# Raph1821/Matcha-TTS-etu-UPMC-ENSAM

Hardware: AMD Instinct MI355X
Metric: training utterances/sec (whole node) + maximum_path Mcells/sec, LJSpeech batch=32 (higher is better)
Workload: dtype bf16; 1 GPU; MatchaTTS train step (encoder + MAS + CFM decoder fwd/bwd + clip + AdamW), B=32/GPU, Tx=120, Ty=600, 80 mels; model=MatchaTTS(n_vocab=150, out_channels=80, hidden_channels=192), global_batch=32, seq_len=600, text_len=120, parallelism=dp1, precision=bf16-parity, hip_graph=True, weight_planes=2, text_encoder_forward=fp32fwd (backward bf16)

## Files before the change

### matcha-tts-etu-upmc-ensam_amd/csrc/losses.hip

```cpp
#include <hip/hip_runtime.h>

#include <cmath>
#include <cstdint>

#include "mtts_common.h"

namespace {

constexpr int kLT = 64;
constexpr int kLThreads = 256;
constexpr int kLMaxC = 128;
constexpr int kLPitch = kLMaxC + 1;

__device__ __forceinline__ float block_sum(float v, float *red) {
#pragma unroll
    for (int off = 32; off > 0; off >>= 1) v += __shfl_xor(v, off);
    __syncthreads();
    if ((threadIdx.x & 63) == 0) red[threadIdx.x >> 6] = v;
    __syncthreads();
    float s = 0.f;
    if (threadIdx.x == 0) {
#pragma unroll
        for (int i = 0; i < kLThreads / 64; ++i) s += red[i];
    }
    return s;
}

__global__ __launch_bounds__(kLThreads) void loss_partials_kernel(const float *__restrict__ u_pred,
                                                                   const float *__restrict__ x1,
                                                                   const float *__restrict__ z,
                                                                   const float *__restrict__ y,
                                                                   const float *__restrict__ mu_y,
                                                                   const float *__restrict__ mask, int C,
                                                                   int T, float one_minus_sigma,
                                                                   float *__restrict__ partials) {
    __shared__ float su[kLT * kLPitch];
    __shared__ float red[kLThreads / 64];
    const int b = blockIdx.y, t0 = blockIdx.x * kLT;
    const int nt = min(kLT, T - t0);
    const float *mb = mask + (size_t)b * T + t0;
    const size_t cm = (size_t)b * C * T;
    float d_acc = 0.f, p_acc = 0.f;
    if (u_pred) {
        const float *ub = u_pred + ((size_t)b * T + t0) * C;
#pragma unroll 4
        for (int e = threadIdx.x; e < nt * C; e += kLThreads) {
            const int tl = e / C, c = e - tl * C;
            su[tl * kLPitch + c] = ub[e];
        }
        __syncthreads();
    }
#pragma unroll 4
    for (int e = threadIdx.x; e < C * kLT; e += kLThreads) {
        const int c = e / kLT, tl = e - c * kLT;
        if (tl >= nt) continue;
        const size_t i = cm + (size_t)c * T + t0 + tl;
        if (u_pred) {
            const float u = x1[i] - one_minus_sigma * z[i];
            const float d = su[tl * kLPitch + c] - u;
            d_acc = fmaf(d, d, d_acc);
        }
        if (mu_y) {
            const float d = y[i] - mu_y[i];
            p_acc += 0.5f * (d * d + 1.8378770664093453f) * mb[tl];
        }
    }
    const float ds = block_sum(d_acc, red);
    const float ps = block_sum(p_acc, red);
    if (threadIdx.x == 0) {
        const size_t blk = (size_t)blockIdx.y * gridDim.x + blockIdx.x;
        partials[2 * blk] = ds;
        partials[2 * blk + 1] = ps;
    }
}

__global__ __launch_bounds__(kLThreads) void loss_finalize_kernel(const float *__restrict__ partials, int nblk,
                                                                   const float *__restrict__ mask, int BT,
                                                                   int C, float *__restrict__ out) {
    __shared__ float red[kLThreads / 64];
    float d = 0.f, p = 0.f, m = 0.f;
    for (int i = threadIdx.x; i < nblk; i += kLThreads) {
        d += partials[2 * i];
        p += partials[2 * i + 1];
    }
    for (int i = threadIdx.x; i < BT; i += kLThreads) m += mask[i];
    d = block_sum(d, red);
    p = block_sum(p, red);
    m = block_sum(m, red);
    if (threadIdx.x == 0) {
        const float denom = m * (float)C;
        out[0] = d / denom;
        out[1] = p / denom;
        out[2] = denom;
    }
}

__global__ __launch_bounds__(kLThreads) void loss_bwd_kernel(const float *__restrict__ g_diff,
                                                              const float *__restrict__ g_prior,
                                                              const float *__restrict__ denom_p,
                                                              const float *__restrict__ u_pred,
                                                              const float *__restrict__ x1, const float *__restrict__ z,
                                                              const float *__restrict__ y,
                                                              const float *__restrict__ mu_y,
                                                              const float *__restrict__ mask, int C, int T,
                                                              float one_minus_sigma, float *__restrict__ du_pred,
                                                              float *__restrict__ dmu_y) {
    __shared__ float su[kLT * kLPitch];
    const int b = blockIdx.y, t0 = blockIdx.x * kLT;
    const int nt = min(kLT, T - t0);
    const float *mb = mask + (size_t)b * T + t0;
    const size_t cm = (size_t)b * C * T;
    const float denom = denom_p[0];
    if (du_pred) {
    #pragma unroll 4
    for (int e = threadIdx.x; e < C * kLT; e += kLThreads) {
            const int c = e / kLT, tl = e - c * kLT;
            if (tl < nt) {
                const size_t i = cm + (size_t)c * T + t0 + tl;
                su[tl * kLPitch + c] = x1[i] - one_minus_sigma * z[i];
            }
        }
        __syncthreads();
        const float g = 2.f * g_diff[0] / denom;
        const size_t tb = ((size_t)b * T + t0) * C;
#pragma unroll 4
        for (int e = threadIdx.x; e < nt * C; e += kLThreads) {
            const int tl = e / C, c = e - tl * C;
            du_pred[tb + e] = g * (u_pred[tb + e] - su[tl * kLPitch + c]);
        }
    }
    if (dmu_y) {
        const float g = -g_prior[0] / denom;
    #pragma unroll 4
    for (int e = threadIdx.x; e < C * kLT; e += kLThreads) {
            const int c = e / kLT, tl = e - c * kLT;
            if (tl >= nt) continue;
            const size_t i = cm + (size_t)c * T + t0 + tl;
            dmu_y[i] = g * (y[i] - mu_y[i]) * mb[tl];
        }
    }
}

}

extern "C" size_t mtts_losses_workspace_size(int32_t B, int32_t T) {
    if (B < 0 || T < 0) return 0;
    return (size_t)B * ((T + kLT - 1) / kLT) * 2 * sizeof(float);
}

extern "C" int mtts_losses_fwd(const float *u_pred, const float *x1, const float *z, const float *y,
                               const float *mu_y, const float *mask, int32_t B, int32_t C, int32_t T,
                               float sigma_min, float *out, void *workspace, size_t workspace_bytes,
                               void *hip_stream) {
    MTTS_CHECK_ARG(mask && out && B >= 1 && T >= 1 && C >= 1 && B <= 65535, "losses_fwd: bad args");
    MTTS_CHECK_ARG(C <= kLMaxC, "losses_fwd: C > 128");
    MTTS_CHECK_ARG(!u_pred || (x1 && z), "losses_fwd: the CFM loss needs x1 and z");
    MTTS_CHECK_ARG(!mu_y || y, "losses_fwd: the prior loss needs y");
    if (!workspace || workspace_bytes < mtts_losses_workspace_size(B, T))
        return mtts::fail(MTTS_ERR_WORKSPACE, "losses_fwd: workspace too small");
    hipStream_t st = static_cast<hipStream_t>(hip_stream);
    dim3 grid((T + kLT - 1) / kLT, B);
    float *part = static_cast<float *>(workspace);
    hipLaunchKernelGGL(loss_partials_kernel, grid, dim3(kLThreads), 0, st, u_pred, x1, z, y, mu_y, mask, C, T,
                       (float)(1.0 - (double)sigma_min), part);
    int rc = mtts::check_launch("loss_partials_kernel");
    if (rc) return rc;
    hipLaunchKernelGGL(loss_finalize_kernel, dim3(1), dim3(kLThreads), 0, st, part, (int)(grid.x * grid.y), mask,
                       B * T, C, out);
    return mtts::check_launch("loss_finalize_kernel");
}

extern "C" int mtts_losses_bwd(const float *g_diff, const float *g_prior, const float *fwd_out, const float *u_pred, const float *x1,
                               const float *z, const float *y, const float *mu_y, const float *mask,
                               int32_t B, int32_t C, int32_t T, float sigma_min, float *du_pred, float *dmu_y,
                               void *hip_stream) {
    MTTS_CHECK_ARG(fwd_out && mask && B >= 1 && T >= 1 && C >= 1 && B <= 65535 && C <= kLMaxC,
                   "losses_bwd: bad args");
    MTTS_CHECK_ARG(!du_pred || (g_diff && u_pred && x1 && z), "losses_bwd: du_pred needs g_diff, u_pred, x1, z");
    MTTS_CHECK_ARG(!dmu_y || (g_prior && y && mu_y), "losses_bwd: dmu_y needs g_prior, y, mu_y");
    if (!du_pred && !dmu_y) return MTTS_OK;
    dim3 grid((T + kLT - 1) / kLT, B);
    hipLaunchKernelGGL(loss_bwd_kernel, grid, dim3(kLThreads), 0, static_cast<hipStream_t>(hip_stream), g_diff,
                       g_prior, fwd_out + 2, u_pred, x1, z, y, mu_y, mask, C, T, (float)(1.0 - (double)sigma_min), du_pred,
                       dmu_y);
    return mtts::check_launch("loss_bwd_kernel");
}

namespace {

constexpr int kGThreads = 1024;

__global__ __launch_bounds__(256) void sequence_mask_kernel(const int64_t *__restrict__ lengths, int B, int T,
                                                            float *__restrict__ mask, float *__restrict__ key_bias) {
    const int64_t i = (int64_t)blockIdx.x * 256 + threadIdx.x;
    if (i >= (int64_t)B * T) return;
    const int b = (int)(i / T), t = (int)(i - (int64_t)b * T);
    const float m = (int64_t)t < lengths[b] ? 1.f : 0.f;
    if (mask) mask[i] = m;
    if (key_bias) key_bias[i] = (m - 1.0f) * 1e4f;
}

__device__ __forceinline__ float big_block_sum(float v, float *red) {
#pragma unroll
    for (int off = 32; off > 0; off >>= 1) v += __shfl_xor(v, off);
    __syncthreads();
    if ((threadIdx.x & 63) == 0) red[threadIdx.x >> 6] = v;
    __syncthreads();
    float s = 0.f;
    if (threadIdx.x == 0) {
#pragma unroll
        for (int i = 0; i < kGThreads / 64; ++i) s += red[i];
    }
    return s;
}

__device__ __forceinline__ float dur_diff(const float *logw, const float *dur, const int64_t *lengths, int T, int64_t i) {
    const int b = (int)(i / T), t = (int)(i - (int64_t)b * T);
    const float m = (int64_t)t < lengths[b] ? 1.f : 0.f;
    const float target = logf(1e-8f + dur[i]) * m;
    return logw[i] - target;
}

__global__ __launch_bounds__(kGThreads) void duration_loss_fwd_kernel(const float *__restrict__ logw,
                                                                      const float *__restrict__ dur,
                                                                      const int64_t *__restrict__ lengths, int B, int T,
                                                                      float *__restrict__ out) {
    __shared__ float red[kGThreads / 64];
    float acc = 0.f;
    for (int64_t i = threadIdx.x; i < (int64_t)B * T; i += kGThreads) {
        const float d = dur_diff(logw, dur, lengths, T, i);
        acc += d * d;
    }
    const float s = big_block_sum(acc, red);
    if (threadIdx.x == 0) {
        int64_t l = 0;
        for (int b = 0; b < B; ++b) l += lengths[b];
        const float L = (float)l;
        out[0] = s / L;
        out[1] = L;
    }
}

__global__ __launch_bounds__(256) void duration_loss_bwd_kernel(const float *__restrict__ g,
                                                                const float *__restrict__ fwd_out,
                                                                const float *__restrict__ logw,
                                                                const float *__restrict__ dur,
                                                                const int64_t *__restrict__ lengths, int B, int T,
                                                                float *__restrict__ dlogw) {
    const int64_t i = (int64_t)blockIdx.x * 256 + threadIdx.x;
    if (i >= (int64_t)B * T) return;
    const float gl = g[0] / fwd_out[1];
    const float d = dur_diff(logw, dur, lengths, T, i);
    dlogw[i] = gl * (2.0f * d);
}

__global__ void loss_sum_kernel(const float *__restrict__ dur, const float *__restrict__ prior,
                                const float *__restrict__ diff, float *__restrict__ total, float *__restrict__ logged) {
    if (threadIdx.x != 0) return;
    const float d = dur[0], p = prior ? prior[0] : 0.f, f = diff[0];
    const float t = (d + p) + f;
    total[0] = t;
    if (logged) {
        logged[0] = d;
        logged[1] = p;
        logged[2] = f;
        logged[3] = t;
    }
// ... 39 lines not shown
```

### matcha-tts-etu-upmc-ensam_amd/csrc/time_mlp.hip

```cpp
#include <hip/hip_runtime.h>

#include <cmath>
#include <cstdint>
#include <cstdlib>

#include "mtts_common.h"
#include "mtts_decoder.h"

namespace {

typedef float f32x16 __attribute__((ext_vector_type(16)));
constexpr int kChunk = 64;

enum Mode { kFwd = 0, kDgrad = 1, kWgrad = 2 };

struct MatTable {
    const float *W[MTTS_ROWS_MAX_MATS];
    const float *bias[MTTS_ROWS_MAX_MATS];
    float *out[MTTS_ROWS_MAX_MATS];
    float *out2[MTTS_ROWS_MAX_MATS];
    const float *dy[MTTS_ROWS_MAX_MATS];
    int N[MTTS_ROWS_MAX_MATS];
    int n_off[MTTS_ROWS_MAX_MATS + 1];
    int r_off[MTTS_ROWS_MAX_MATS + 1];
    int nmat;
};

__device__ __forceinline__ float act_fwd(int act, float v) {
    if (act == MTTS_ROWS_ACT_SILU) return v / (1.0f + expf(-v));
    if (act == MTTS_ROWS_ACT_MISH) {
        if (v >= 15.f) return v;
        const float e = expf(v), n = e * (e + 2.f);
        return v * n / (n + 2.f);
    }
    return v;
}

__device__ __forceinline__ float act_grad(int act, float v) {
    if (act == MTTS_ROWS_ACT_SILU) {
        const float s = 1.0f / (1.0f + expf(-v));
        return s * (1.0f + v * (1.0f - s));
    }
    if (act == MTTS_ROWS_ACT_MISH) {
        if (v >= 15.f) return 1.f;
        const float e = expf(v), n = e * (e + 2.f), t = n / (n + 2.f), s = e / (1.f + e);
        return t + v * s * (1.f - t * t);
    }
    return 1.f;
}

constexpr int kWaves = 4;
constexpr int kRange = kWaves * kChunk;
constexpr int kLd = 65;

struct Ws {
    float *part;
    unsigned *counter;
    int ks;
    int passes;
};

template <int MODE>
__global__ __launch_bounds__(64 * kWaves) void rows_gemm_kernel(MatTable T, const float *__restrict__ x, int B, int K,
                                                                int act, const float *__restrict__ pre,
                                                                float *__restrict__ dx, int col_tiles, Ws ws) {
    extern __shared__ float lds[];
    const int lane = threadIdx.x & 63, wave = threadIdx.x >> 6;
    const int lr = lane & 31, s = lane >> 5;
    const int tile = blockIdx.x / ws.ks, ksi = blockIdx.x - tile * ws.ks;
    const int rt = tile / col_tiles, ct = tile - rt * col_tiles;
    int mat = 0, m0 = rt * 32, c0 = ct * 32, R = 0;
    if constexpr (MODE == kFwd) {
        while (mat + 1 < T.nmat && c0 >= T.n_off[mat + 1]) ++mat;
        c0 -= T.n_off[mat];
        R = K;
    } else if constexpr (MODE == kDgrad) {
        R = T.r_off[T.nmat];
    } else {
        while (mat + 1 < T.nmat && m0 >= T.n_off[mat + 1]) ++mat;
        m0 -= T.n_off[mat];
        R = B;
    }
    float *sA = lds + wave * 2 * 32 * kLd, *sB = sA + 32 * kLd;
    auto stage = [&](const float *base, int ld, int nrows, int r0, int r_end, float *dst) {
#pragma unroll
        for (int q = 0; q < 8; ++q) {
            const int e = q * 64 + lane, row = e >> 4, c4 = (e & 15) * 4;
            float4 v = make_float4(0.f, 0.f, 0.f, 0.f);
            if (row < nrows && r0 + c4 < r_end) v = *reinterpret_cast<const float4 *>(base + (size_t)row * ld + r0 + c4);
            dst[row * kLd + c4] = v.x;
            dst[row * kLd + c4 + 1] = v.y;
            dst[row * kLd + c4 + 2] = v.z;
            dst[row * kLd + c4 + 3] = v.w;
        }
    };
    f32x16 acc;
#pragma unroll
    for (int v = 0; v < 16; ++v) acc[v] = 0.f;
    for (int pass = 0; pass < ws.passes; ++pass) {
        const int r0 = (ksi * ws.passes + pass) * kRange + wave * kChunk;
        if (pass > 0) __syncthreads();
        float a[32], b[32];
        if constexpr (MODE == kFwd) {
            stage(x + (size_t)m0 * K, K, min(32, B - m0), r0, R, sA);
            stage(T.W[mat] + (size_t)c0 * K, K, min(32, T.N[mat] - c0), r0, R, sB);
            __syncthreads();
#pragma unroll
            for (int j = 0; j < 32; ++j) {
                a[j] = sA[lr * kLd + 32 * s + j];
                b[j] = sB[lr * kLd + 32 * s + j];
            }
        } else if constexpr (MODE == kDgrad) {
            int dm = 0;
            while (dm + 1 < T.nmat && r0 >= T.r_off[dm + 1]) ++dm;
            const int base = T.r_off[dm], Nm = T.N[dm];
            stage(T.dy[dm] + (size_t)m0 * Nm - base, Nm, min(32, B - m0), r0, min(R, base + Nm), sA);
            __syncthreads();
            const int k = c0 + lr;
#pragma unroll
            for (int j = 0; j < 32; ++j) {
                const int r = r0 + 32 * s + j;
                a[j] = sA[lr * kLd + 32 * s + j];
                b[j] = r - base < Nm && k < K ? T.W[dm][(size_t)(r - base) * K + k] : 0.f;
            }
        } else {
            const int n = m0 + lr, k = c0 + lr, Nm = T.N[mat];
#pragma unroll
            for (int j = 0; j < 32; ++j) {
                const int r = r0 + 32 * s + j;
                a[j] = r < R && n < Nm ? T.dy[mat][(size_t)r * Nm + n] : 0.f;
                b[j] = r < R && k < K ? x[(size_t)r * K + k] : 0.f;
            }
        }
#pragma unroll
        for (int j = 0; j < 32; ++j) acc = __builtin_amdgcn_mfma_f32_32x32x2f32(a[j], b[j], acc, 0, 0, 0);
    }
    const int nw = blockDim.x >> 6;
    if (nw > 1) {
        __syncthreads();
        float *part = lds;
        if (wave > 0) {
#pragma unroll
            for (int v = 0; v < 16; ++v) part[(wave * 16 + v) * 64 + lane] = acc[v];
        }
        __syncthreads();
        if (wave > 0) return;
        for (int w = 1; w < nw; ++w)
#pragma unroll
            for (int v = 0; v < 16; ++v) acc[v] += part[(w * 16 + v) * 64 + lane];
    }
    if (ws.ks > 1) {
        float *mine = ws.part + ((size_t)tile * ws.ks + ksi) * 1024;
#pragma unroll
        for (int v = 0; v < 16; ++v) mine[v * 64 + lane] = acc[v];
        __threadfence();
        unsigned ticket = 0;
        if (lane == 0) ticket = atomicAdd(ws.counter + tile, 1u);
        ticket = __shfl(ticket, 0);
        if (ticket != (unsigned)ws.ks - 1) return;
        __threadfence();
        const float *all = ws.part + (size_t)tile * ws.ks * 1024;
#pragma unroll
        for (int v = 0; v < 16; ++v) acc[v] = __builtin_nontemporal_load(all + v * 64 + lane);
        for (int q = 1; q < ws.ks; ++q)
#pragma unroll
            for (int v = 0; v < 16; ++v) acc[v] += __builtin_nontemporal_load(all + (size_t)q * 1024 + v * 64 + lane);
        if (lane == 0) atomicExch(ws.counter + tile, 0u);
    }
#pragma unroll
    for (int v = 0; v < 16; ++v) {
        const int row = m0 + (v & 3) + 8 * (v >> 2) + 4 * s, col = c0 + lr;
        if constexpr (MODE == kFwd) {
            const int N = T.N[mat];
            if (row < B && col < N) {
                const float o = acc[v] + (T.bias[mat] ? T.bias[mat][col] : 0.f);
                T.out[mat][(size_t)row * N + col] = o;
                if (T.out2[mat]) T.out2[mat][(size_t)row * N + col] = act_fwd(act, o);
            }
        } else if constexpr (MODE == kDgrad) {
            if (row < B && col < K) {
                const size_t o = (size_t)row * K + col;
                dx[o] = pre ? acc[v] * act_grad(act, pre[o]) : acc[v];
            }
        } else {
            if (row < T.N[mat] && col < K) T.out[mat][(size_t)row * K + col] = acc[v];
        }
    }
    if constexpr (MODE == kWgrad) {
        if (ct == 0 && T.out2[mat] && lane < 32 && m0 + lane < T.N[mat]) {
            const int n = m0 + lane, Nm = T.N[mat];
            float sacc = 0.f;
            for (int b2 = 0; b2 < B; ++b2) sacc += T.dy[mat][(size_t)b2 * Nm + n];
            T.out2[mat][n] = sacc;
        }
    }
}

int fill_table(MatTable &T, int nmat, const int32_t *N) {
    MTTS_CHECK_ARG(nmat >= 1 && nmat <= MTTS_ROWS_MAX_MATS && N, "rows_linear: 1..8 matrices");
    T.nmat = nmat;
    T.n_off[0] = T.r_off[0] = 0;
    for (int i = 0; i < nmat; ++i) {
        MTTS_CHECK_ARG(N[i] >= 1, "rows_linear: N_i >= 1");
        T.N[i] = N[i];
        T.n_off[i + 1] = T.n_off[i] + (N[i] + 31) / 32 * 32;
        T.r_off[i + 1] = T.r_off[i] + (N[i] + kChunk - 1) / kChunk * kChunk;
    }
    return MTTS_OK;
}

struct Geo {
    int ks, waves, passes;
    size_t lds;
};
int passes_of(int R) {
    const char *e = getenv("MTTS_ROWS_PASSES");
    const int want = e ? atoi(e) : 1, need = (R + kRange - 1) / kRange;
    return want < 1 ? 1 : (want > need ? need : want);
}

Geo geometry(int R, bool staged) {
    Geo g;
    g.passes = passes_of(R);
    g.ks = (R + kRange * g.passes - 1) / (kRange * g.passes);
    g.waves = R >= kRange ? kWaves : (R + kChunk - 1) / kChunk;
    const size_t stage = staged ? (size_t)g.waves * 2 * 32 * kLd * sizeof(float) : 0;
    const size_t red = g.waves > 1 ? (size_t)g.waves * 16 * 64 * sizeof(float) : 0;
    g.lds = stage > red ? stage : red;
    return g;
}

int check_ws(const Geo &g, int tiles, void *ws, size_t ws_bytes, Ws &w) {
    w.ks = g.ks;
    w.passes = g.passes;
    w.part = nullptr;
    w.counter = nullptr;
    if (g.ks == 1) return MTTS_OK;
    const size_t need = mtts::align_up((size_t)tiles * sizeof(unsigned), 256) + (size_t)tiles * g.ks * 1024 * sizeof(float);
    if (!ws || ws_bytes < need || (uintptr_t)ws % 256)
        return mtts::fail(MTTS_ERR_WORKSPACE, "rows_linear: workspace too small (mtts_rows_linear_workspace_size)");
    w.counter = static_cast<unsigned *>(ws);
    w.part = reinterpret_cast<float *>(static_cast<char *>(ws) + mtts::align_up((size_t)tiles * sizeof(unsigned), 256));
    return MTTS_OK;
}

}

extern "C" size_t mtts_rows_linear_workspace_size(int32_t B, int32_t K, int32_t nmat, const int32_t *N) {
    if (B < 1 || K < 1 || nmat < 1 || nmat > MTTS_ROWS_MAX_MATS || !N) return 0;
    size_t nt = 0, nr = 0;
    for (int i = 0; i < nmat; ++i) {
        nt += (size_t)(N[i] + 31) / 32;
        nr += (size_t)(N[i] + kChunk - 1) / kChunk * kChunk;
    }
    const size_t rt = (size_t)(B + 31) / 32, kt = (size_t)(K + 31) / 32;
    auto ks = [](size_t r) { return (r + kRange - 1) / kRange; };
    const size_t t[3] = {rt * nt, rt * kt, nt * kt}, k[3] = {ks(K), ks(nr), ks(B)};
    size_t tiles = 0, parts = 0;
    for (int m = 0; m < 3; ++m) {
        if (k[m] < 2) continue;
        tiles = t[m] > tiles ? t[m] : tiles;
        parts = t[m] * k[m] > parts ? t[m] * k[m] : parts;
    }
    return mtts::align_up(tiles * sizeof(unsigned), 256) + parts * 1024 * sizeof(float);
}

extern "C" int mtts_rows_linear_fwd(const float *x, int32_t B, int32_t K, int32_t nmat, const float *const *W,
                                    const float *const *bias, const int32_t *N, float *const *out,
                                    float *const *out_act, int32_t act, void *workspace, size_t workspace_bytes,
                                    void *hip_stream) {
    MTTS_CHECK_ARG(x && W && out && B >= 1 && K >= 4 && K % 4 == 0 && (uintptr_t)x % 16 == 0,
                   "rows_linear_fwd: bad args (K % 4 == 0, 16-byte aligned rows)");
    MTTS_CHECK_ARG(act >= MTTS_ROWS_ACT_NONE && act <= MTTS_ROWS_ACT_MISH, "rows_linear_fwd: bad act");
    MatTable T{};
    if (int rc = fill_table(T, nmat, N)) return rc;
    int col_tiles = 0;
    for (int i = 0; i < nmat; ++i) {
        MTTS_CHECK_ARG(W[i] && out[i] && (uintptr_t)W[i] % 16 == 0, "rows_linear_fwd: null / unaligned matrix");
        T.W[i] = W[i];
        T.bias[i] = bias ? bias[i] : nullptr;
        T.out[i] = out[i];
        T.out2[i] = out_act ? out_act[i] : nullptr;
        col_tiles += (N[i] + 31) / 32;
    }
    const int tiles = ((B + 31) / 32) * col_tiles;
    const Geo g = geometry(K, true);
    Ws w;
    if (int rc = check_ws(g, tiles, workspace, workspace_bytes, w)) return rc;
    hipLaunchKernelGGL(rows_gemm_kernel<kFwd>, dim3(tiles * g.ks), dim3(64 * g.waves), g.lds,
                       static_cast<hipStream_t>(hip_stream), T, x, B, K, act, nullptr, nullptr, col_tiles, w);
    return mtts::check_launch("rows_gemm_kernel<fwd>");
}

extern "C" int mtts_rows_linear_bwd(const float *a, const float *pre, int32_t act, int32_t B, int32_t K, int32_t nmat,
                                    const float *const *W, const int32_t *N, const float *const *dy, float *dx,
                                    float *const *dW, float *const *db, void *workspace, size_t workspace_bytes,
                                    void *hip_stream) {
    MTTS_CHECK_ARG(W && dy && B >= 1 && K >= 1, "rows_linear_bwd: bad args");
    MTTS_CHECK_ARG(act >= MTTS_ROWS_ACT_NONE && act <= MTTS_ROWS_ACT_MISH && (act == MTTS_ROWS_ACT_NONE || pre),
                   "rows_linear_bwd: act' needs the pre-activation");
    MTTS_CHECK_ARG(!dW || a, "rows_linear_bwd: dW needs the input rows");
    hipStream_t st = static_cast<hipStream_t>(hip_stream);
    MatTable T{};
    if (int rc = fill_table(T, nmat, N)) return rc;
    int row_tiles = 0;
    for (int i = 0; i < nmat; ++i) {
        MTTS_CHECK_ARG(W[i] && dy[i] && (!dx || (N[i] % 4 == 0 && (uintptr_t)dy[i] % 16 == 0)),
                       "rows_linear_bwd: null matrix (dx: N_i % 4 == 0, 16-byte aligned dy rows)");
        T.W[i] = W[i];
        T.dy[i] = dy[i];
        T.out[i] = dW ? dW[i] : nullptr;
        T.out2[i] = db ? db[i] : nullptr;
        MTTS_CHECK_ARG(!dW || dW[i], "rows_linear_bwd: null dW");
        row_tiles += (N[i] + 31) / 32;
    }
    const int kt = (K + 31) / 32;
    if (dx) {
        const int tiles = ((B + 31) / 32) * kt;
        const Geo g = geometry(T.r_off[nmat], true);
        Ws w;
        if (int rc = check_ws(g, tiles, workspace, workspace_bytes, w)) return rc;
        hipLaunchKernelGGL(rows_gemm_kernel<kDgrad>, dim3(tiles * g.ks), dim3(64 * g.waves), g.lds, st, T, nullptr, B,
                           K, act, pre, dx, kt, w);
        if (int rc = mtts::check_launch("rows_gemm_kernel<dgrad>")) return rc;
    }
    if (dW) {
        const Geo g = geometry(B, false);
        Ws w;
        if (int rc = check_ws(g, row_tiles * kt, workspace, workspace_bytes, w)) return rc;
        hipLaunchKernelGGL(rows_gemm_kernel<kWgrad>, dim3(row_tiles * kt * g.ks), dim3(64 * g.waves), g.lds, st, T, a,
                           B, K, act, nullptr, nullptr, kt, w);
        if (int rc = mtts::check_launch("rows_gemm_kernel<wgrad>")) return rc;
    }
    return MTTS_OK;
}
```

Measured before the change: 4570 utterances/s.

## Restructure loss kernels with register prefetch and merge rows-linear backward passes

The loss forward and backward kernels now give each thread a fixed token and a strided set of channels, prefetch x1/z/y/mu_y into registers, and load u_pred with float4 reads walked through LDS. The forward kernel also computes the mask sum per block, so the finalize kernel no longer rescans the whole mask. In time_mlp, the templated rows GEMM is split into a dedicated forward kernel and a single fused backward kernel that handles both dgrad and wgrad tiles in one launch, which drops the env-controlled split-K backward path and its workspace. The goal is fewer launches and more coalesced or vectorised memory traffic, at the cost of more registers per thread and a substantially rewritten GEMM backward whose correctness must be re-verified.

After: 4583 utterances/s, median of 6. No clear change (+0.3%).

```diff
diff --git a/matcha-tts-etu-upmc-ensam_amd/csrc/losses.hip b/matcha-tts-etu-upmc-ensam_amd/csrc/losses.hip
--- a/matcha-tts-etu-upmc-ensam_amd/csrc/losses.hip
+++ b/matcha-tts-etu-upmc-ensam_amd/csrc/losses.hip
@@ -11,6 +11,8 @@
 constexpr int kLThreads = 256;
 constexpr int kLMaxC = 128;
 constexpr int kLPitch = kLMaxC + 1;
+constexpr int kLVec = kLT * kLMaxC / 4 / kLThreads;
+constexpr int kLFin = 8;
 
 __device__ __forceinline__ float block_sum(float v, float *red) {
 #pragma unroll
@@ -26,64 +28,132 @@
     return s;
 }
 
+struct TokenWalk {
+    int e, tl, c, dq, dr;
+    __device__ __forceinline__ TokenWalk(int C) {
+        e = threadIdx.x * 4;
+        tl = e / C;
+        c = e - tl * C;
+        dq = (kLThreads * 4) / C;
+        dr = kLThreads * 4 - dq * C;
+    }
+    __device__ __forceinline__ void next(int C) {
+        e += kLThreads * 4;
+        tl += dq;
+        c += dr;
+        if (c >= C) {
+            c -= C;
+            ++tl;
+        }
+    }
+};
+
+template <int NI>
 __global__ __launch_bounds__(kLThreads) void loss_partials_kernel(const float *__restrict__ u_pred,
                                                                    const float *__restrict__ x1,
                                                                    const float *__restrict__ z,
                                                                    const float *__restrict__ y,
                                                                    const float *__restrict__ mu_y,
                                                                    const float *__restrict__ mask, int C,
-                                                                   int T, float one_minus_sigma,
+                                                                   int T, float one_minus_sigma, int vec,
                                                                    float *__restrict__ partials) {
     __shared__ float su[kLT * kLPitch];
     __shared__ float red[kLThreads / 64];
     const int b = blockIdx.y, t0 = blockIdx.x * kLT;
     const int nt = min(kLT, T - t0);
-    const float *mb = mask + (size_t)b * T + t0;
-    const size_t cm = (size_t)b * C * T;
+    const int tl = threadIdx.x & 63, w = threadIdx.x >> 6;
+    const bool live = tl < nt;
+    const float mv = live ? mask[(size_t)b * T + t0 + tl] : 0.f;
+    const size_t cm = (size_t)b * C * T + t0 + tl;
+    const bool y_is_x1 = u_pred && y == x1;
+    const float *ub = u_pred ? u_pred + ((size_t)b * T + t0) * C : nullptr;
+    float4 vu[kLVec];
+    if (u_pred && vec) {
+        TokenWalk tw(C);
+#pragma unroll
+        for (int k = 0; k < kLVec; ++k, tw.next(C))
+            if (tw.e < nt * C) vu[k] = *reinterpret_cast<const float4 *>(ub + tw.e);
+    }
+    float vx[NI], vz[NI], vy[NI], vm[NI];
+#pragma unroll
+    for (int i = 0; i < NI; ++i) {
+        const int c = w + 4 * i;
+        const bool ok = live && c < C;
+        const size_t idx = cm + (size_t)c * T;
+        vx[i] = ok && u_pred ? x1[idx] : 0.f;
+        vz[i] = ok && u_pred ? z[idx] : 0.f;
+        vy[i] = ok && mu_y && !y_is_x1 ? y[idx] : 0.f;
+        vm[i] = ok && mu_y ? mu_y[idx] : 0.f;
+    }
+    if (u_pred) {
+        if (vec) {
+            TokenWalk tw(C);
+#pragma unroll
+            for (int k = 0; k < kLVec; ++k, tw.next(C)) {
+                if (tw.e < nt * C) {
+                    float *d = su + tw.tl * kLPitch + tw.c;
+                    d[0] = vu[k].x, d[1] = vu[k].y, d[2] = vu[k].z, d[3] = vu[k].w;
+                }
+            }
+        } else {
+            for (int e = threadIdx.x; e < nt * C; e += kLThreads) {
+                const int t2 = e / C, c = e - t2 * C;
+                su[t2 * kLPitch + c] = ub[e];
+            }
+        }
+        __syncthreads();
+    }
     float d_acc = 0.f, p_acc = 0.f;
-    if (u_pred) {
-        const float *ub = u_pred + ((size_t)b * T + t0) * C;
-#pragma unroll 4
-        for (int e = threadIdx.x; e < nt * C; e += kLThreads) {
-            const int tl = e / C, c = e - tl * C;
-            su[tl * kLPitch + c] = ub[e];
-        }
-        __syncthreads();
-    }
-#pragma unroll 4
-    for (int e = threadIdx.x; e < C * kLT; e += kLThreads) {
-        const int c = e / kLT, tl = e - c * kLT;
-        if (tl >= nt) continue;
-        const size_t i = cm + (size_t)c * T + t0 + tl;
+#pragma unroll
+    for (int i = 0; i < NI; ++i) {
+        const int c = w + 4 * i;
+        if (!(live && c < C)) continue;
         if (u_pred) {
-            const float u = x1[i] - one_minus_sigma * z[i];
+            const float u = vx[i] - one_minus_sigma * vz[i];
             const float d = su[tl * kLPitch + c] - u;
             d_acc = fmaf(d, d, d_acc);
         }
         if (mu_y) {
-            const float d = y[i] - mu_y[i];
-            p_acc += 0.5f * (d * d + 1.8378770664093453f) * mb[tl];
-        }
-    }
+            const float d = (y_is_x1 ? vx[i] : vy[i]) - vm[i];
+            p_acc += 0.5f * (d * d + 1.8378770664093453f) * mv;
+        }
+    }
+    float ms = mv;
+#pragma unroll
+    for (int off = 32; off > 0; off >>= 1) ms += __shfl_xor(ms, off);
     const float ds = block_sum(d_acc, red);
     const float ps = block_sum(p_acc, red);
     if (threadIdx.x == 0) {
         const size_t blk = (size_t)blockIdx.y * gridDim.x + blockIdx.x;
-        partials[2 * blk] = ds;
-        partials[2 * blk + 1] = ps;
-    }
-}
-
-__global__ __launch_bounds__(kLThreads) void loss_finalize_kernel(const float *__restrict__ partials, int nblk,
-                                                                   const float *__restrict__ mask, int BT,
-                                                                   int C, float *__restrict__ out) {
+        partials[3 * blk] = ds;
+        partials[3 * blk + 1] = ps;
+        partials[3 * blk + 2] = ms;
+    }
+}
+
+__global__ __launch_bounds__(kLThreads) void loss_finalize_kernel(const float *__restrict__ partials, int nblk, int C,
+                                                                   float *__restrict__ out) {
     __shared__ float red[kLThreads / 64];
     float d = 0.f, p = 0.f, m = 0.f;
-    for (int i = threadIdx.x; i < nblk; i += kLThreads) {
-        d += partials[2 * i];
-        p += partials[2 * i + 1];
-    }
-    for (int i = threadIdx.x; i < BT; i += kLThreads) m += mask[i];
+    for (int base = threadIdx.x; base < nblk; base += kLThreads * kLFin) {
+        float pd[kLFin], pp[kLFin], pm[kLFin];
+#pragma unroll
+        for (int k = 0; k < kLFin; ++k) {
+            const int i = base + k * kLThreads;
+            const bool ok = i < nblk;
+            pd[k] = ok ? partials[3 * (size_t)i] : 0.f;
+            pp[k] = ok ? partials[3 * (size_t)i + 1] : 0.f;
+            pm[k] = ok ? partials[3 * (size_t)i + 2] : 0.f;
+        }
+#pragma unroll
+        for (int k = 0; k < kLFin; ++k) {
+            if (base + k * kLThreads < nblk) {
+                d += pd[k];
+                p += pp[k];
+                m += pm[k];
+            }
+        }
+    }
     d = block_sum(d, red);
     p = block_sum(p, red);
     m = block_sum(m, red);
@@ -95,6 +165,7 @@
     }
 }
 
+template <int NI>
 __global__ __launch_bounds__(kLThreads) void loss_bwd_kernel(const float *__restrict__ g_diff,
                                                               const float *__restrict__ g_prior,
                                                               const float *__restrict__ denom_p,
@@ -103,49 +174,83 @@
                                                               const float *__restrict__ y,
                                                               const float *__restrict__ mu_y,
                                                               const float *__restrict__ mask, int C, int T,
-                                                              float one_minus_sigma, float *__restrict__ du_pred,
+                                                              float one_minus_sigma, int vec, float *__restrict__ du_pred,
                                                               float *__restrict__ dmu_y) {
     __shared__ float su[kLT * kLPitch];
     const int b = blockIdx.y, t0 = blockIdx.x * kLT;
     const int nt = min(kLT, T - t0);
-    const float *mb = mask + (size_t)b * T + t0;
-    const size_t cm = (size_t)b * C * T;
+    const int tl = threadIdx.x & 63, w = threadIdx.x >> 6;
+    const bool live = tl < nt;
     const float denom = denom_p[0];
+    const float gd = du_pred ? g_diff[0] : 0.f, gp = dmu_y ? g_prior[0] : 0.f;
+    const float mv = live && dmu_y ? mask[(size_t)b * T + t0 + tl] : 0.f;
+    const size_t cm = (size_t)b * C * T + t0 + tl;
+    const size_t tb = ((size_t)b * T + t0) * C;
+    const bool y_is_x1 = du_pred && y == x1;
+    float4 vu[kLVec];
+    if (du_pred && vec) {
+        TokenWalk tw(C);
+#pragma unroll
+        for (int k = 0; k < kLVec; ++k, tw.next(C))
+            if (tw.e < nt * C) vu[k] = *reinterpret_cast<const float4 *>(u_pred + tb + tw.e);
+    }
+    float vx[NI], vz[NI], vy[NI], vm[NI];
+#pragma unroll
+    for (int i = 0; i < NI; ++i) {
+        const int c = w + 4 * i;
+        const bool ok = live && c < C;
+        const size_t idx = cm + (size_t)c * T;
+        vx[i] = ok && du_pred ? x1[idx] : 0.f;
+        vz[i] = ok && du_pred ? z[idx] : 0.f;
+        vy[i] = ok && dmu_y && !y_is_x1 ? y[idx] : 0.f;
+        vm[i] = ok && dmu_y ? mu_y[idx] : 0.f;
+    }
+    if (dmu_y) {
+        const float g = -gp / denom;
+#pragma unroll
+        for (int i = 0; i < NI; ++i) {
+            const int c = w + 4 * i;
+            if (live && c < C) dmu_y[cm + (size_t)c * T] = g * ((y_is_x1 ? vx[i] : vy[i]) - vm[i]) * mv;
+        }
+    }
     if (du_pred) {
-    #pragma unroll 4
-    for (int e = threadIdx.x; e < C * kLT; e += kLThreads) {
-            const int c = e / kLT, tl = e - c * kLT;
-            if (tl < nt) {
-                const size_t i = cm + (size_t)c * T + t0 + tl;
-                su[tl * kLPitch + c] = x1[i] - one_minus_sigma * z[i];
+#pragma unroll
+        for (int i = 0; i < NI; ++i) {
+            const int c = w + 4 * i;
+            if (live && c < C) su[tl * kLPitch + c] = vx[i] - one_minus_sigma * vz[i];
+        }
+        __syncthreads();
+        const float g = 2.f * gd / denom;
+        if (vec) {
+            TokenWalk tw(C);
+#pragma unroll
+            for (int k = 0; k < kLVec; ++k, tw.next(C)) {
+                if (tw.e < nt * C) {
+                    const float *s = su + tw.tl * kLPitch + tw.c;
+                    float4 o;
+                    o.x = g * (vu[k].x - s[0]);
+                    o.y = g * (vu[k].y - s[1]);
+                    o.z = g * (vu[k].z - s[2]);
+                    o.w = g * (vu[k].w - s[3]);
+                    *reinterpret_cast<float4 *>(du_pred + tb + tw.e) = o;
+                }
             }
-        }
-        __syncthreads();
-        const float g = 2.f * g_diff[0] / denom;
-        const size_t tb = ((size_t)b * T + t0) * C;
-#pragma unroll 4
-        for (int e = threadIdx.x; e < nt * C; e += kLThreads) {
-            const int tl = e / C, c = e - tl * C;
-            du_pred[tb + e] = g * (u_pred[tb + e] - su[tl * kLPitch + c]);
-        }
-    }
-    if (dmu_y) {
-        const float g = -g_prior[0] / denom;
-    #pragma unroll 4
-    for (int e = threadIdx.x; e < C * kLT; e += kLThreads) {
-            const int c = e / kLT, tl = e - c * kLT;
-            if (tl >= nt) continue;
-            const size_t i = cm + (size_t)c * T + t0 + tl;
-            dmu_y[i] = g * (y[i] - mu_y[i]) * mb[tl];
-        }
-    }
-}
+        } else {
+            for (int e = threadIdx.x; e < nt * C; e += kLThreads) {
+                const int t2 = e / C, c = e - t2 * C;
+                du_pred[tb + e] = g * (u_pred[tb + e] - su[t2 * kLPitch + c]);
+            }
+        }
+    }
+}
+
+bool aligned16(const void *p) { return (reinterpret_cast<uintptr_t>(p) & 15) == 0; }
 
 }
 
 extern "C" size_t mtts_losses_workspace_size(int32_t B, int32_t T) {
     if (B < 0 || T < 0) return 0;
-    return (size_t)B * ((T + kLT - 1) / kLT) * 2 * sizeof(float);
+    return (size_t)B * ((T + kLT - 1) / kLT) * 3 * sizeof(float);
 }
 
 extern "C" int mtts_losses_fwd(const float *u_pred, const float *x1, const float *z, const float *y,
@@ -161,12 +266,17 @@
     hipStream_t st = static_cast<hipStream_t>(hip_stream);
     dim3 grid((T + kLT - 1) / kLT, B);
     float *part = static_cast<float *>(workspace);
-    hipLaunchKernelGGL(loss_partials_kernel, grid, dim3(kLThreads), 0, st, u_pred, x1, z, y, mu_y, mask, C, T,
-                       (float)(1.0 - (double)sigma_min), part);
+    const float oms = (float)(1.0 - (double)sigma_min);
+    const int vec = C % 4 == 0 && aligned16(u_pred);
+    if (C <= 80)
+        hipLaunchKernelGGL(loss_partials_kernel<20>, grid, dim3(kLThreads), 0, st, u_pred, x1, z, y, mu_y, mask, C, T,
+                           oms, vec, part);
+    else
+        hipLaunchKernelGGL(loss_partials_kernel<kLMaxC / 4>, grid, dim3(kLThreads), 0, st, u_pred, x1, z, y, mu_y,
+                           mask, C, T, oms, vec, part);
     int rc = mtts::check_launch("loss_partials_kernel");
     if (rc) return rc;
-    hipLaunchKernelGGL(loss_finalize_kernel, dim3(1), dim3(kLThreads), 0, st, part, (int)(grid.x * grid.y), mask,
-                       B * T, C, out);
+    hipLaunchKernelGGL(loss_finalize_kernel, dim3(1), dim3(kLThreads), 0, st, part, (int)(grid.x * grid.y), C, out);
     return mtts::check_launch("loss_finalize_kernel");
 }
 
@@ -179,10 +289,16 @@
     MTTS_CHECK_ARG(!du_pred || (g_diff && u_pred && x1 && z), "losses_bwd: du_pred needs g_diff, u_pred, x1, z");
     MTTS_CHECK_ARG(!dmu_y || (g_prior && y && mu_y), "losses_bwd: dmu_y needs g_prior, y, mu_y");
     if (!du_pred && !dmu_y) return MTTS_OK;
+    hipStream_t st = static_cast<hipStream_t>(hip_stream);
     dim3 grid((T + kLT - 1) / kLT, B);
-    hipLaunchKernelGGL(loss_bwd_kernel, grid, dim3(kLThreads), 0, static_cast<hipStream_t>(hip_stream), g_diff,
-                       g_prior, fwd_out + 2, u_pred, x1, z, y, mu_y, mask, C, T, (float)(1.0 - (double)sigma_min), du_pred,
-                       dmu_y);
+    const float oms = (float)(1.0 - (double)sigma_min);
+    const int vec = C % 4 == 0 && aligned16(u_pred) && aligned16(du_pred);
+    if (C <= 80)
+        hipLaunchKernelGGL(loss_bwd_kernel<20>, grid, dim3(kLThreads), 0, st, g_diff, g_prior, fwd_out + 2, u_pred, x1,
+                           z, y, mu_y, mask, C, T, oms, vec, du_pred, dmu_y);
+    else
+        hipLaunchKernelGGL(loss_bwd_kernel<kLMaxC / 4>, grid, dim3(kLThreads), 0, st, g_diff, g_prior, fwd_out + 2,
+                           u_pred, x1, z, y, mu_y, mask, C, T, oms, vec, du_pred, dmu_y);
     return mtts::check_launch("loss_bwd_kernel");
 }
 
diff --git a/matcha-tts-etu-upmc-ensam_amd/csrc/time_mlp.hip b/matcha-tts-etu-upmc-ensam_amd/csrc/time_mlp.hip
--- a/matcha-tts-etu-upmc-ensam_amd/csrc/time_mlp.hip
+++ b/matcha-tts-etu-upmc-ensam_amd/csrc/time_mlp.hip
@@ -2,7 +2,6 @@
 
 #include <cmath>
 #include <cstdint>
-#include <cstdlib>
 
 #include "mtts_common.h"
 #include "mtts_decoder.h"
@@ -11,8 +10,6 @@
 
 typedef float f32x16 __attribute__((ext_vector_type(16)));
 constexpr int kChunk = 64;
-
-enum Mode { kFwd = 0, kDgrad = 1, kWgrad = 2 };
 
 struct MatTable {
     const float *W[MTTS_ROWS_MAX_MATS];
@@ -57,37 +54,25 @@
     float *part;
     unsigned *counter;
     int ks;
-    int passes;
 };
 
-template <int MODE>
-__global__ __launch_bounds__(64 * kWaves) void rows_gemm_kernel(MatTable T, const float *__restrict__ x, int B, int K,
-                                                                int act, const float *__restrict__ pre,
-                                                                float *__restrict__ dx, int col_tiles, Ws ws) {
+__global__ __launch_bounds__(64 * kWaves) void rows_gemm_fwd_kernel(MatTable T, const float *__restrict__ x, int B,
+                                                                    int K, int act, int col_tiles, Ws ws) {
     extern __shared__ float lds[];
     const int lane = threadIdx.x & 63, wave = threadIdx.x >> 6;
     const int lr = lane & 31, s = lane >> 5;
     const int tile = blockIdx.x / ws.ks, ksi = blockIdx.x - tile * ws.ks;
     const int rt = tile / col_tiles, ct = tile - rt * col_tiles;
-    int mat = 0, m0 = rt * 32, c0 = ct * 32, R = 0;
-    if constexpr (MODE == kFwd) {
-        while (mat + 1 < T.nmat && c0 >= T.n_off[mat + 1]) ++mat;
-        c0 -= T.n_off[mat];
-        R = K;
-    } else if constexpr (MODE == kDgrad) {
-        R = T.r_off[T.nmat];
-    } else {
-        while (mat + 1 < T.nmat && m0 >= T.n_off[mat + 1]) ++mat;
-        m0 -= T.n_off[mat];
-        R = B;
-    }
+    int mat = 0, m0 = rt * 32, c0 = ct * 32;
+    while (mat + 1 < T.nmat && c0 >= T.n_off[mat + 1]) ++mat;
+    c0 -= T.n_off[mat];
     float *sA = lds + wave * 2 * 32 * kLd, *sB = sA + 32 * kLd;
-    auto stage = [&](const float *base, int ld, int nrows, int r0, int r_end, float *dst) {
+    auto stage = [&](const float *base, int nrows, int r0, float *dst) {
 #pragma unroll
         for (int q = 0; q < 8; ++q) {
             const int e = q * 64 + lane, row = e >> 4, c4 = (e & 15) * 4;
             float4 v = make_float4(0.f, 0.f, 0.f, 0.f);
-            if (row < nrows && r0 + c4 < r_end) v = *reinterpret_cast<const float4 *>(base + (size_t)row * ld + r0 + c4);
+            if (row < nrows && r0 + c4 < K) v = *reinterpret_cast<const float4 *>(base + (size_t)row * K + r0 + c4);
             dst[row * kLd + c4] = v.x;
             dst[row * kLd + c4 + 1] = v.y;
             dst[row * kLd + c4 + 2] = v.z;
@@ -97,44 +82,18 @@
     f32x16 acc;
 #pragma unroll
     for (int v = 0; v < 16; ++v) acc[v] = 0.f;
-    for (int pass = 0; pass < ws.passes; ++pass) {
-        const int r0 = (ksi * ws.passes + pass) * kRange + wave * kChunk;
-        if (pass > 0) __syncthreads();
-        float a[32], b[32];
-        if constexpr (MODE == kFwd) {
-            stage(x + (size_t)m0 * K, K, min(32, B - m0), r0, R, sA);
-            stage(T.W[mat] + (size_t)c0 * K, K, min(32, T.N[mat] - c0), r0, R, sB);
-            __syncthreads();
-#pragma unroll
-            for (int j = 0; j < 32; ++j) {
-                a[j] = sA[lr * kLd + 32 * s + j];
-                b[j] = sB[lr * kLd + 32 * s + j];
-            }
-        } else if constexpr (MODE == kDgrad) {
-            int dm = 0;
-            while (dm + 1 < T.nmat && r0 >= T.r_off[dm + 1]) ++dm;
-            const int base = T.r_off[dm], Nm = T.N[dm];
-            stage(T.dy[dm] + (size_t)m0 * Nm - base, Nm, min(32, B - m0), r0, min(R, base + Nm), sA);
-            __syncthreads();
-            const int k = c0 + lr;
-#pragma unroll
-            for (int j = 0; j < 32; ++j) {
-                const int r = r0 + 32 * s + j;
-                a[j] = sA[lr * kLd + 32 * s + j];
-                b[j] = r - base < Nm && k < K ? T.W[dm][(size_t)(r - base) * K + k] : 0.f;
-            }
-        } else {
-            const int n = m0 + lr, k = c0 + lr, Nm = T.N[mat];
-#pragma unroll
-            for (int j = 0; j < 32; ++j) {
-                const int r = r0 + 32 * s + j;
-                a[j] = r < R && n < Nm ? T.dy[mat][(size_t)r * Nm + n] : 0.f;
-                b[j] = r < R && k < K ? x[(size_t)r * K + k] : 0.f;
-            }
-        }
-#pragma unroll
-        for (int j = 0; j < 32; ++j) acc = __builtin_amdgcn_mfma_f32_32x32x2f32(a[j], b[j], acc, 0, 0, 0);
-    }
+    const int r0 = ksi * kRange + wave * kChunk;
+    stage(x + (size_t)m0 * K, min(32, B - m0), r0, sA);
+    stage(T.W[mat] + (size_t)c0 * K, min(32, T.N[mat] - c0), r0, sB);
+    __syncthreads();
+    float a[32], b[32];
+#pragma unroll
+    for (int j = 0; j < 32; ++j) {
+        a[j] = sA[lr * kLd + 32 * s + j];
+        b[j] = sB[lr * kLd + 32 * s + j];
+    }
+#pragma unroll
+    for (int j = 0; j < 32; ++j) acc = __builtin_amdgcn_mfma_f32_32x32x2f32(a[j], b[j], acc, 0, 0, 0);
     const int nw = blockDim.x >> 6;
     if (nw > 1) {
         __syncthreads();
@@ -167,31 +126,195 @@
             for (int v = 0; v < 16; ++v) acc[v] += __builtin_nontemporal_load(all + (size_t)q * 1024 + v * 64 + lane);
         if (lane == 0) atomicExch(ws.counter + tile, 0u);
     }
+    const int N = T.N[mat];
 #pragma unroll
     for (int v = 0; v < 16; ++v) {
         const int row = m0 + (v & 3) + 8 * (v >> 2) + 4 * s, col = c0 + lr;
-        if constexpr (MODE == kFwd) {
-            const int N = T.N[mat];
-            if (row < B && col < N) {
-                const float o = acc[v] + (T.bias[mat] ? T.bias[mat][col] : 0.f);
-                T.out[mat][(size_t)row * N + col] = o;
-                if (T.out2[mat]) T.out2[mat][(size_t)row * N + col] = act_fwd(act, o);
+        if (row < B && col < N) {
+            const float o = acc[v] + (T.bias[mat] ? T.bias[mat][col] : 0.f);
+            T.out[mat][(size_t)row * N + col] = o;
+            if (T.out2[mat]) T.out2[mat][(size_t)row * N + col] = act_fwd(act, o);
+        }
+    }
+}
+
+constexpr int kMaxWaves = 8;
+constexpr int kLdB = 33;
+constexpr int kStage = 64 * kLdB;
+static_assert(kStage >= 32 * kLd, "staging slot holds either block shape");
+
+struct Pick {
+    const float *W, *dy;
+    float *out, *out2;
+    int N, base;
+};
+__device__ __forceinline__ Pick pick(const MatTable &T, const int *off, int i) {
+    Pick p{T.W[0], T.dy[0], T.out[0], T.out2[0], T.N[0], 0};
+#pragma unroll
+    for (int m = 1; m < MTTS_ROWS_MAX_MATS; ++m)
+        if (m < T.nmat && i >= off[m]) p = Pick{T.W[m], T.dy[m], T.out[m], T.out2[m], T.N[m], off[m]};
+    return p;
+}
+
+__device__ __forceinline__ void wgrad_tile(const Pick &P, const float *__restrict__ a, int B, int K, int m0, int c0,
+                                           bool with_bias, int lane) {
+    const int lr = lane & 31, s = lane >> 5;
+    const int n = m0 + lr, k = c0 + lr, Nm = P.N;
+    const bool bias_lane = with_bias && P.out2 && lane < 32 && n < Nm;
+    f32x16 tot, grp;
+    float sacc = 0.f;
+    const int chunks = (B + kChunk - 1) / kChunk;
+    for (int c = 0; c < chunks; ++c) {
+        const int r0 = c * kChunk + 32 * s;
+        float fa[32], fb[32], bv[32];
+#pragma unroll
+        for (int j = 0; j < 32; ++j) {
+            const int r = r0 + j;
+            fa[j] = r < B && n < Nm ? P.dy[(size_t)r * Nm + n] : 0.f;
+            fb[j] = r < B && k < K ? a[(size_t)r * K + k] : 0.f;
+        }
+        if (bias_lane) {
+#pragma unroll
+            for (int h = 0; h < 2; ++h) {
+#pragma unroll
+                for (int j = 0; j < 32; ++j) {
+                    const int r = c * kChunk + 32 * h + j;
+                    bv[j] = r < B ? P.dy[(size_t)r * Nm + n] : 0.f;
+                }
+#pragma unroll
+                for (int j = 0; j < 32; ++j)
+                    if (c * kChunk + 32 * h + j < B) sacc += bv[j];
             }
-        } else if constexpr (MODE == kDgrad) {
-            if (row < B && col < K) {
-                const size_t o = (size_t)row * K + col;
-                dx[o] = pre ? acc[v] * act_grad(act, pre[o]) : acc[v];
+        }
+        f32x16 acc;
+#pragma unroll
+        for (int v = 0; v < 16; ++v) acc[v] = 0.f;
+#pragma unroll
+        for (int j = 0; j < 32; ++j) acc = __builtin_amdgcn_mfma_f32_32x32x2f32(fa[j], fb[j], acc, 0, 0, 0);
+        if ((c & 3) == 0) {
+            grp = acc;
+        } else {
+#pragma unroll
+            for (int v = 0; v < 16; ++v) grp[v] += acc[v];
+        }
+        if ((c & 3) == 3 || c == chunks - 1) {
+            if (c < 4) {
+                tot = grp;
+            } else {
+#pragma unroll
+                for (int v = 0; v < 16; ++v) tot[v] += grp[v];
             }
-        } else {
-            if (row < T.N[mat] && col < K) T.out[mat][(size_t)row * K + col] = acc[v];
-        }
-    }
-    if constexpr (MODE == kWgrad) {
-        if (ct == 0 && T.out2[mat] && lane < 32 && m0 + lane < T.N[mat]) {
-            const int n = m0 + lane, Nm = T.N[mat];
-            float sacc = 0.f;
-            for (int b2 = 0; b2 < B; ++b2) sacc += T.dy[mat][(size_t)b2 * Nm + n];
-            T.out2[mat][n] = sacc;
+        }
+    }
+#pragma unroll
+    for (int v = 0; v < 16; ++v) {
+        const int row = m0 + (v & 3) + 8 * (v >> 2) + 4 * s;
+        if (row < Nm && k < K) P.out[(size_t)row * K + k] = tot[v];
+    }
+    if (bias_lane) P.out2[n] = sacc;
+}
+
+__global__ __launch_bounds__(64 * kMaxWaves) void rows_gemm_bwd_kernel(MatTable T, const float *__restrict__ a, int B,
+                                                                       int K, int act, const float *__restrict__ pre,
+                                                                       float *__restrict__ dx, int kt, int d_tiles,
+                                                                       int w_tiles) {
+    extern __shared__ float lds[];
+    const int lane = threadIdx.x & 63, wave = __builtin_amdgcn_readfirstlane(threadIdx.x >> 6);
+    const int nw = blockDim.x >> 6;
+    if ((int)blockIdx.x >= d_tiles) {
+        const int tile = ((int)blockIdx.x - d_tiles) * nw + wave;
+        if (tile >= w_tiles) return;
+        const int rt = tile / kt, ct = tile - rt * kt;
+        const Pick P = pick(T, T.n_off, rt * 32);
+        wgrad_tile(P, a, B, K, rt * 32 - P.base, ct * 32, ct == 0, lane);
+        return;
+    }
+    const int lr = lane & 31, s = lane >> 5;
+    const int rt = (int)blockIdx.x / kt, ct = (int)blockIdx.x - rt * kt;
+    const int m0 = rt * 32, c0 = ct * 32, R = T.r_off[T.nmat];
+    const int chunks = R / kChunk, rounds = (chunks + nw - 1) / nw;
+    float *sA = lds + wave * 2 * kStage, *sB = sA + kStage;
+    float *part = lds;
+
+    float4 va[8], vb[8];
+    auto gload = [&](int round) {
+        const int r0 = (round * nw + wave) * kChunk;
+        const Pick D = pick(T, T.r_off, r0);
+        const float *ab = D.dy + (size_t)m0 * D.N - D.base;
+        const float *bb = D.W + (size_t)(r0 - D.base) * K + c0;
+        const int a_rows = min(32, B - m0), a_end = min(R, D.base + D.N);
+        const int b_rows = D.N - (r0 - D.base);
+#pragma unroll
+        for (int q = 0; q < 8; ++q) {
+            const int e = q * 64 + lane, row = e >> 4, c4 = (e & 15) * 4, br = e >> 3, bc = (e & 7) * 4;
+            va[q] = vb[q] = make_float4(0.f, 0.f, 0.f, 0.f);
+            if (r0 < R && row < a_rows && r0 + c4 < a_end)
+                va[q] = *reinterpret_cast<const float4 *>(ab + (size_t)row * D.N + r0 + c4);
+            if (r0 < R && br < b_rows && c0 + bc < K) vb[q] = *reinterpret_cast<const float4 *>(bb + (size_t)br * K + bc);
+        }
+    };
+    auto put = [](float *dst, float4 v) {
+        dst[0] = v.x;
+        dst[1] = v.y;
+        dst[2] = v.z;
+        dst[3] = v.w;
+    };
+
+    constexpr int kOwn = 16;
+    float tot[kOwn];
+    gload(0);
+    for (int round = 0; round < rounds; ++round) {
+        const bool active = (round * nw + wave) * kChunk < R;
+        if (round > 0) __syncthreads();
+#pragma unroll
+        for (int q = 0; q < 8; ++q) {
+            const int e = q * 64 + lane;
+            put(sA + (e >> 4) * kLd + (e & 15) * 4, va[q]);
+            put(sB + (e >> 3) * kLdB + (e & 7) * 4, vb[q]);
+        }
+        if (round + 1 < rounds) gload(round + 1);
+        __syncthreads();
+        f32x16 acc;
+#pragma unroll
+        for (int v = 0; v < 16; ++v) acc[v] = 0.f;
+        if (active) {
+            float fa[32], fb[32];
+#pragma unroll
+            for (int j = 0; j < 32; ++j) {
+                fa[j] = sA[lr * kLd + 32 * s + j];
+                fb[j] = sB[(32 * s + j) * kLdB + lr];
+            }
+#pragma unroll
+            for (int j = 0; j < 32; ++j) acc = __builtin_amdgcn_mfma_f32_32x32x2f32(fa[j], fb[j], acc, 0, 0, 0);
+        }
+        __syncthreads();
+        if (active) {
+#pragma unroll
+            for (int v = 0; v < 16; ++v) part[(wave * 16 + v) * 64 + lane] = acc[v];
+        }
+        __syncthreads();
+        const int live = min(nw, chunks - round * nw);
+#pragma unroll
+        for (int i = 0; i < kOwn; ++i) {
+            const int e = (int)threadIdx.x + i * (int)blockDim.x;
+            if (e < 1024) {
+                for (int g = 0; g < live; g += 4) {
+                    float grp = part[g * 1024 + e];
+                    for (int w = g + 1; w < min(g + 4, live); ++w) grp += part[w * 1024 + e];
+                    tot[i] = (round == 0 && g == 0) ? grp : tot[i] + grp;
+                }
+            }
+        }
+    }
+#pragma unroll
+    for (int i = 0; i < kOwn; ++i) {
+        const int e = (int)threadIdx.x + i * (int)blockDim.x;
+        if (e >= 1024) continue;
+        const int v = e >> 6, el = e & 63;
+        const int row = m0 + (v & 3) + 8 * (v >> 2) + 4 * (el >> 5), col = c0 + (el & 31);
+        if (row < B && col < K) {
+            const size_t o = (size_t)row * K + col;
+            dx[o] = pre ? tot[i] * act_grad(act, pre[o]) : tot[i];
         }
     }
 }
@@ -209,60 +332,18 @@
     return MTTS_OK;
 }
 
-struct Geo {
-    int ks, waves, passes;
-    size_t lds;
-};
-int passes_of(int R) {
-    const char *e = getenv("MTTS_ROWS_PASSES");
-    const int want = e ? atoi(e) : 1, need = (R + kRange - 1) / kRange;
-    return want < 1 ? 1 : (want > need ? need : want);
-}
-
-Geo geometry(int R, bool staged) {
-    Geo g;
-    g.passes = passes_of(R);
-    g.ks = (R + kRange * g.passes - 1) / (kRange * g.passes);
-    g.waves = R >= kRange ? kWaves : (R + kChunk - 1) / kChunk;
-    const size_t stage = staged ? (size_t)g.waves * 2 * 32 * kLd * sizeof(float) : 0;
-    const size_t red = g.waves > 1 ? (size_t)g.waves * 16 * 64 * sizeof(float) : 0;
-    g.lds = stage > red ? stage : red;
-    return g;
-}
-
-int check_ws(const Geo &g, int tiles, void *ws, size_t ws_bytes, Ws &w) {
-    w.ks = g.ks;
-    w.passes = g.passes;
-    w.part = nullptr;
-    w.counter = nullptr;
-    if (g.ks == 1) return MTTS_OK;
-    const size_t need = mtts::align_up((size_t)tiles * sizeof(unsigned), 256) + (size_t)tiles * g.ks * 1024 * sizeof(float);
-    if (!ws || ws_bytes < need || (uintptr_t)ws % 256)
-        return mtts::fail(MTTS_ERR_WORKSPACE, "rows_linear: workspace too small (mtts_rows_linear_workspace_size)");
-    w.counter = static_cast<unsigned *>(ws);
-    w.part = reinterpret_cast<float *>(static_cast<char *>(ws) + mtts::align_up((size_t)tiles * sizeof(unsigned), 256));
-    return MTTS_OK;
-}
+int fwd_splits(int K) { return (K + kRange - 1) / kRange; }
+int fwd_waves(int K) { return K >= kRange ? kWaves : (K + kChunk - 1) / kChunk; }
 
 }
 
 extern "C" size_t mtts_rows_linear_workspace_size(int32_t B, int32_t K, int32_t nmat, const int32_t *N) {
     if (B < 1 || K < 1 || nmat < 1 || nmat > MTTS_ROWS_MAX_MATS || !N) return 0;
-    size_t nt = 0, nr = 0;
-    for (int i = 0; i < nmat; ++i) {
-        nt += (size_t)(N[i] + 31) / 32;
-        nr += (size_t)(N[i] + kChunk - 1) / kChunk * kChunk;
-    }
-    const size_t rt = (size_t)(B + 31) / 32, kt = (size_t)(K + 31) / 32;
-    auto ks = [](size_t r) { return (r + kRange - 1) / kRange; };
-    const size_t t[3] = {rt * nt, rt * kt, nt * kt}, k[3] = {ks(K), ks(nr), ks(B)};
-    size_t tiles = 0, parts = 0;
-    for (int m = 0; m < 3; ++m) {
-        if (k[m] < 2) continue;
-        tiles = t[m] > tiles ? t[m] : tiles;
-        parts = t[m] * k[m] > parts ? t[m] * k[m] : parts;
-    }
-    return mtts::align_up(tiles * sizeof(unsigned), 256) + parts * 1024 * sizeof(float);
+    if (fwd_splits(K) < 2) return 0;
+    size_t tiles = 0;
+    for (int i = 0; i < nmat; ++i) tiles += (size_t)(N[i] + 31) / 32;
+    tiles *= (size_t)(B + 31) / 32;
+    return mtts::align_up(tiles * sizeof(unsigned), 256) + tiles * fwd_splits(K) * 1024 * sizeof(float);
 }
 
 extern "C" int mtts_rows_linear_fwd(const float *x, int32_t B, int32_t K, int32_t nmat, const float *const *W,
@@ -283,30 +364,43 @@
         T.out2[i] = out_act ? out_act[i] : nullptr;
         col_tiles += (N[i] + 31) / 32;
     }
-    const int tiles = ((B + 31) / 32) * col_tiles;
-    const Geo g = geometry(K, true);
-    Ws w;
-    if (int rc = check_ws(g, tiles, workspace, workspace_bytes, w)) return rc;
-    hipLaunchKernelGGL(rows_gemm_kernel<kFwd>, dim3(tiles * g.ks), dim3(64 * g.waves), g.lds,
-                       static_cast<hipStream_t>(hip_stream), T, x, B, K, act, nullptr, nullptr, col_tiles, w);
-    return mtts::check_launch("rows_gemm_kernel<fwd>");
+    const int tiles = ((B + 31) / 32) * col_tiles, waves = fwd_waves(K);
+    Ws w{nullptr, nullptr, fwd_splits(K)};
+    if (w.ks > 1) {
+        const size_t counters = mtts::align_up((size_t)tiles * sizeof(unsigned), 256);
+        if (!workspace || workspace_bytes < counters + (size_t)tiles * w.ks * 1024 * sizeof(float) ||
+            (uintptr_t)workspace % 256)
+            return mtts::fail(MTTS_ERR_WORKSPACE, "rows_linear: workspace too small (mtts_rows_linear_workspace_size)");
+        w.counter = static_cast<unsigned *>(workspace);
+        w.part = reinterpret_cast<float *>(static_cast<char *>(workspace) + counters);
+    }
+    const size_t lds = (size_t)waves * 2 * 32 * kLd * sizeof(float);
+    if (lds > 64 * 1024 &&
+        hipFuncSetAttribute(reinterpret_cast<const void *>(rows_gemm_fwd_kernel),
+                            hipFuncAttributeMaxDynamicSharedMemorySize, (int)lds) != hipSuccess)
+        return mtts::fail(MTTS_ERR_HIP, "rows_linear_fwd: cannot reserve the staging LDS");
+    hipLaunchKernelGGL(rows_gemm_fwd_kernel, dim3(tiles * w.ks), dim3(64 * waves), lds,
+                       static_cast<hipStream_t>(hip_stream), T, x, B, K, act, col_tiles, w);
+    return mtts::check_launch("rows_gemm_fwd_kernel");
 }
 
 extern "C" int mtts_rows_linear_bwd(const float *a, const float *pre, int32_t act, int32_t B, int32_t K, int32_t nmat,
                                     const float *const *W, const int32_t *N, const float *const *dy, float *dx,
                                     float *const *dW, float *const *db, void *workspace, size_t workspace_bytes,
                                     void *hip_stream) {
+    (void)workspace, (void)workspace_bytes;
     MTTS_CHECK_ARG(W && dy && B >= 1 && K >= 1, "rows_linear_bwd: bad args");
     MTTS_CHECK_ARG(act >= MTTS_ROWS_ACT_NONE && act <= MTTS_ROWS_ACT_MISH && (act == MTTS_ROWS_ACT_NONE || pre),
                    "rows_linear_bwd: act' needs the pre-activation");
     MTTS_CHECK_ARG(!dW || a, "rows_linear_bwd: dW needs the input rows");
-    hipStream_t st = static_cast<hipStream_t>(hip_stream);
+    MTTS_CHECK_ARG(!dx || K % 4 == 0, "rows_linear_bwd: dx needs K % 4 == 0");
     MatTable T{};
     if (int rc = fill_table(T, nmat, N)) return rc;
     int row_tiles = 0;
     for (int i = 0; i < nmat; ++i) {
-        MTTS_CHECK_ARG(W[i] && dy[i] && (!dx || (N[i] % 4 == 0 && (uintptr_t)dy[i] % 16 == 0)),
-                       "rows_linear_bwd: null matrix (dx: N_i % 4 == 0, 16-byte aligned dy rows)");
+        MTTS_CHECK_ARG(W[i] && dy[i] &&
+                           (!dx || (N[i] % 4 == 0 && (uintptr_t)dy[i] % 16 == 0 && (uintptr_t)W[i] % 16 == 0)),
+                       "rows_linear_bwd: null matrix (dx: N_i % 4 == 0, 16-byte aligned dy and W rows)");
         T.W[i] = W[i];
         T.dy[i] = dy[i];
         T.out[i] = dW ? dW[i] : nullptr;
@@ -314,23 +408,17 @@
         MTTS_CHECK_ARG(!dW || dW[i], "rows_linear_bwd: null dW");
         row_tiles += (N[i] + 31) / 32;
     }
+    if (!dx && !dW) return MTTS_OK;
     const int kt = (K + 31) / 32;
-    if (dx) {
-        const int tiles = ((B + 31) / 32) * kt;
-        const Geo g = geometry(T.r_off[nmat], true);
-        Ws w;
-        if (int rc = check_ws(g, tiles, workspace, workspace_bytes, w)) return rc;
-        hipLaunchKernelGGL(rows_gemm_kernel<kDgrad>, dim3(tiles * g.ks), dim3(64 * g.waves), g.lds, st, T, nullptr, B,
-                           K, act, pre, dx, kt, w);
-        if (int rc = mtts::check_launch("rows_gemm_kernel<dgrad>")) return rc;
-    }
-    if (dW) {
-        const Geo g = geometry(B, false);
-        Ws w;
-        if (int rc = check_ws(g, row_tiles * kt, workspace, workspace_bytes, w)) return rc;
-        hipLaunchKernelGGL(rows_gemm_kernel<kWgrad>, dim3(row_tiles * kt * g.ks), dim3(64 * g.waves), g.lds, st, T, a,
-                           B, K, act, nullptr, nullptr, kt, w);
-        if (int rc = mtts::check_launch("rows_gemm_kernel<wgrad>")) return rc;
-    }
-    return MTTS_OK;
-}
+    const int d_tiles = dx ? ((B + 31) / 32) * kt : 0, w_tiles = dW ? row_tiles * kt : 0;
+    const int chunks = T.r_off[nmat] / kChunk;
+    const int waves = dx ? (chunks < kMaxWaves ? chunks : kMaxWaves) : 4;
+    const size_t lds = dx ? (size_t)waves * 2 * kStage * sizeof(float) : 0;
+    if (lds > 64 * 1024 &&
+        hipFuncSetAttribute(reinterpret_cast<const void *>(rows_gemm_bwd_kernel),
+                            hipFuncAttributeMaxDynamicSharedMemorySize, (int)lds) != hipSuccess)
+        return mtts::fail(MTTS_ERR_HIP, "rows_linear_bwd: cannot reserve the staging LDS");
+    hipLaunchKernelGGL(rows_gemm_bwd_kernel, dim3(d_tiles + (w_tiles + waves - 1) / waves), dim3(64 * waves), lds,
+                       static_cast<hipStream_t>(hip_stream), T, a, B, K, act, pre, dx, kt, d_tiles, w_tiles);
+    return mtts::check_launch("rows_gemm_bwd_kernel");
+}
```
